# hpsim/OGL

Measured on AMD Instinct MI355X. Metric: cg_iters_per_sec, higher is better.
Workload: dtype f64

## Files before the change

### ogl_amd/csrc/kernels.hpp

```cpp
#pragma once
#include <hip/hip_runtime.h>

#include "common.hpp"

namespace ogl {

struct DevCriterion {
    double tolerance, rel_tol;
    int32_t min_iter, max_iter, frequency, export_res;
};

struct DevScalars {
    double rho, prev_rho, beta;
    double alpha, omega, gamma;
    double norm_factor;
    double init_res, res;
    double xbar;
    double sums[4];
    int32_t iter;
    int32_t stop;
    int32_t n_evals;
    int32_t stop_phase;
    int32_t stop_turn;
    int32_t comm_error;
// ... 286 lines not shown
void launch_cg_step2(hipStream_t st, int32_t n, double *x, double *r, const double *p,
                     const double *q, const double *inv_diag, double *part_rho, double *part_norm,
                     const DevScalars *s);

struct HaloPutFused;
void launch_cg_step1x(hipStream_t st, int32_t n, double *p, double *x, const double *r,
                      const double *inv_diag, const DevScalars *s, const HaloPutFused *put = nullptr);
void launch_cg_step2r(hipStream_t st, int32_t n, double *r, const double *q, const double *inv_diag,
                      double *part_rho, double *part_norm, const DevScalars *s, double *z_out = nullptr,
                      const HaloPutFused *put = nullptr);

void launch_cg_step1x_fin(hipStream_t st, int32_t n, double *p, double *x, const double *r, const double *inv_diag,
                          const DevScalars *sin, DevScalars *sout, const double *part_rho,
                          const double *part_norm, double *history, int first, const LeadBox &lead = LeadBox{},
                          double *p_out = nullptr, const PRing &ring = PRing{});
void launch_cg_step2r_fin(hipStream_t st, int32_t n, double *r, const double *q, const double *inv_diag,
                          double *part_rho, double *part_norm, const DevScalars *sin, DevScalars *sout,
                          const double *part_beta, double *z_out = nullptr,
                          const LeadBox &lead = LeadBox{});
struct HeldZ {
    unsigned long long *tagged = nullptr;
    int32_t grid = 0;
    int32_t early_slots = 0;
};
constexpr int HZ_B = 4, HZ_R = 11, HZ_L = 9;
int held_z_grid(int *chunks_per_workgroup);
int launch_resident_census(hipStream_t st, int grid, unsigned *arrived, int *out, long long timeout_ticks);
void launch_cg_step2r1x(hipStream_t st, int32_t n, double *r, const double *q, const double *inv_diag, double *p,
                        double *p_out, double *x, DevScalars *s, const double *part_beta, double *history,
                        const LeadBox &lead, const PRing &ring, const HeldZ &hz);
struct HeldQ {
    int32_t on = 0;
    int32_t n_pos = 0;
};
int held_q_positions(const DevSym &A);
int held_q_occupancy(int *per_cu, size_t *lds_bytes);
void launch_cg_turn_held_q(hipStream_t st, const DevSym &A, double *r, const double *inv_diag, double *p, double *p_out,
                           double *x, DevScalars *s, double *history, const LeadBox &lead, const PRing &ring,
                           const HeldZ &hz, const HeldQ &hq);
constexpr int FUSED_FIN_MAX_CHUNKS = 1024;
void launch_cg_turn_sym(hipStream_t st, const DevSym &A, const double *p_in, double *p_out, double *x, const double *z,
                        double *q, double *part_beta, const DevScalars *sin, DevScalars *sout,
                        const double *part_rho, const double *part_norm, double *history, int first,
                        const LeadBox &lead = LeadBox{});
void launch_cg_turn_sym_big(hipStream_t st, const DevSym &A, const double *p_in, double *p_out, double *x,
                            const double *z, double *q, double *part_beta, const DevScalars *s,
                            const HaloFused &hf = HaloFused{}, const double *p_halo_in = nullptr,
                            double *p_halo_out = nullptr);

void launch_gmres_mgs_fold(hipStream_t st, int32_t n, double *w, const double *vprev, double *h_out, const double *vdot,
                           const double *part_in, double *part_out, const DevScalars *gate, const LeadBox &lead = LeadBox{},
                           uint32_t tag = 0);
void launch_bicg_fold1(hipStream_t st, int32_t n, double *p, const double *r, const double *v, const double *inv_diag,
                       double *y, const DevScalars *sin, DevScalars *sout, const double *part_rho,
                       const double *part_norm, double *history, const LeadBox &lead = LeadBox{});
void launch_bicg_fold2(hipStream_t st, int32_t n, const double *r, const double *v, double *sv, const double *inv_diag,
                       double *z, double *part_norm_out, const DevScalars *sin, DevScalars *sout,
                       const double *part_beta, const LeadBox &lead = LeadBox{});
void launch_bicg_fold3(hipStream_t st, int32_t n, double *x, double *r, const double *sv, const double *t,
                       const double *y, const double *z, const double *rr, double *part_rho_out, double *part_norm_out,
                       const DevScalars *sin, DevScalars *sout, const double *part_gamma, const double *part_tt,
                       const double *part_snorm, double *history, int turn, const LeadBox &lead = LeadBox{});
void launch_bicg_step1(hipStream_t st, int32_t n, double *p, const double *r, const double *v,
                       const double *inv_diag, double *y, const DevScalars *s);
void launch_bicg_step2(hipStream_t st, int32_t n, const double *r, const double *v, double *sv,
                       const double *inv_diag, double *z, double *part_norm, const DevScalars *s);
void launch_bicg_step3(hipStream_t st, int32_t n, double *x, double *r, const double *sv,
// ... 140 lines not shown
```

### ogl_amd/csrc/kernels_spmv_sym.hip

```cpp
#include <algorithm>

#include "device_common.hpp"
#include "resident_cg_turn.hpp"

namespace ogl {

namespace {

struct SymOffsets {
    int d[SYM_MAX_OFFSETS];
};
SymOffsets sym_offsets(const DevSym &A, bool *fast)
{
    SymOffsets off;
    for (int j = 0; j < SYM_MAX_OFFSETS; ++j) off.d[j] = A.d[j];
    *fast = A.nd >= 2 && A.d[1] == 1;
    for (int j = 2; j < A.nd; ++j) *fast = *fast && (A.d[j] % 2 == 0);
    return off;
}
template <int MODE, int ND, bool FAST, bool STREAM>
__device__ __forceinline__ double2 sym_rows(int chunk, const RowPair &rp, int n_rows, const SymOffsets &off,
                                            const uint8_t *__restrict__ mask, const double *__restrict__ planes,
                                            const double *__restrict__ x, const double *__restrict__ b,
                                            double2 &xd_out)
// ... 341 lines not shown
        return;
    }
    const unsigned mm = *reinterpret_cast<const unsigned short *>(mask + rp.row);
    const unsigned m0 = mm & 0xffu, m1 = mm >> 8;
    TurnSymRegs<ND> R;
    turn_sym_load<ND, FAST, STREAM>(R, chunk, rp, n_rows, off, planes, p_in, z);
    if (pending) {
        const double beta = s->beta;
        if (beta != 0.0) {
            const double t = s->prev_rho / beta;
            double2 vx = ld2_stream(x, rp);
            vx.x += t * R.vd[0].x;
            vx.y += t * R.vd[0].y;
            st2_stream(x, rp, vx);
        }
    }
    const double rho = s->rho, prev = s->prev_rho;
    const double tmp = (prev == 0.0) ? 0.0 : rho / prev;
    double2 xd;
    double2 acc = turn_sym_rows<ND>(R, m0, m1, tmp, xd);
    st2(p_out, rp, xd);
    if (HALO) {
        __shared__ double ys[CHUNK_ROWS];
        if (hf.chunk_bptr) halo_fused_add<SPMV_PLAIN, true>(hf, chunk, acc.x, acc.y, ys, tmp, ph_in, ph_out);
    }
    st2(q, rp, acc);
    double d = 0.0;
    if (rp.n > 0) d += xd.x * acc.x;
    if (rp.n > 1) d += xd.y * acc.y;
    const double sd = block_sum(d, slot);
    if (threadIdx.x == 0) part_beta[chunk] = sd;
}

struct HeldQSrc {
    static constexpr bool Q_HELD = true;
    static constexpr int STRIDE = 6, WORD = 2;
    int G, n_pos, n_partials;
    const int *__restrict__ block_order;
    __device__ __forceinline__ int chunk_of(int i) const
    {
        const int pos = blockIdx.x + i * G;
        if (pos >= n_pos) return -1;
        const int c = block_order ? block_order[pos] : xcd_chunk(pos);
        return c < n_partials ? c : -1;
    }
};
template <int R, int L, int B, int K, int ND, bool FAST>
__global__ __launch_bounds__(BLOCK, B) void k_cg_turn_held_q(int n, int n_chunks, int n_pos, SymOffsets off,
                                                             const uint8_t *__restrict__ mask,
                                                             const double *__restrict__ planes,
                                                             const int *__restrict__ block_order, double *__restrict__ r,
                                                             const double *__restrict__ inv_diag, double *p, double *p_out,
                                                             double *__restrict__ x, DevScalars *s,
                                                             unsigned long long *tagged, double *history, LeadBox lead,
                                                             const double *p_pend, int ring_phase, int early_slots)
{
    __shared__ double zl[L > 0 ? L * CHUNK_ROWS : 1];
    __shared__ TurnLds lds;
    const TurnScalars ts = turn_prelude<K>(s, ring_phase);
    const TurnArgs a{n, r, inv_diag, p, p_out, x, s, tagged, history, lead, p_pend, early_slots};
    const HeldQSrc src{(int)gridDim.x, n_pos, n_chunks, block_order};
    const int G = gridDim.x, w = blockIdx.x;
    if (ts.stopped) return;
    TurnSlots<R, L> z;
    z.zl = zl;
#pragma unroll
    for (int i = 0; i < R + L; ++i) {
        const int chunk = src.chunk_of(i);
        if (chunk < 0) continue;
        const RowPair rp = my_rows(chunk, n);
        double2 xd;
        double2 vq = sym_rows<SPMV_PLAIN, ND, FAST, true>(chunk, rp, n, off, mask, planes, p, nullptr, xd);
        if (rp.n < 2) vq.y = 0.0;
        if (rp.n < 1) vq.x = 0.0;
        z.put(i, vq);
        double d = 0.0;
        if (rp.n > 0) d += xd.x * vq.x;
        if (rp.n > 1) d += xd.y * vq.y;
        const double sd = block_sum(d, lds.slot);
        if (threadIdx.x == 0) put_tagged(tagged + HeldQSrc::STRIDE * (size_t)chunk, ts.seq, sd);
    }
    const int lead0 = G >= 3 * FIN_WAVES ? 2 * FIN_WAVES : 0;
    if (w >= lead0 && w < lead0 + FIN_WAVES)
        lead_wave_sums_tagged(lead, ts.seq, tagged, HeldQSrc::STRIDE, n_chunks, w - lead0, 0);
    TurnFront<HeldQSrc::Q_HELD> f;
    turn_ask_first(src, a, f);
    double beta;
    if (!turn_await_beta(a, ts, lds, beta)) return;
    resident_cg_turn<R, L, K>(src, a, ts, lds, z, f, beta);
}

}

void launch_spmv_sym(hipStream_t st, const DevSym &A, int mode, const double *x, const double *b, double *y,
                     const SpmvDots &dots, const DevScalars *gate, const HaloFused &hf)
{
    if (A.n_rows == 0) return;
    const int nc = (int)n_chunks(A.n_rows);
    const dim3 grid(A.block_order ? A.n_blocks : xcd_grid(nc)), block(BLOCK);
    bool fast;
    const SymOffsets off = sym_offsets(A, &fast);
#define OGL_SYM_K(MODE, NDOT, ND, FAST, STREAM)                                                                          \
    hipLaunchKernelGGL((k_spmv_sym<MODE, NDOT, ND, FAST, STREAM>), grid, block, 0, st, A.n_rows, nc, off, A.mask, A.planes, \
                       x, b, y, dots.with, dots.part, dots.part_yy, gate, A.block_order, hf)
#define OGL_SYM_ND(MODE, NDOT, ND)                   \
    do {                                             \
        if (fast && A.stream)                        \
            OGL_SYM_K(MODE, NDOT, ND, true, true);   \
        else if (fast)                               \
            OGL_SYM_K(MODE, NDOT, ND, true, false);  \
        else if (A.stream)                           \
            OGL_SYM_K(MODE, NDOT, ND, false, true);  \
        else                                         \
            OGL_SYM_K(MODE, NDOT, ND, false, false); \
    } while (0)
#define OGL_SYM(MODE, NDOT)                    \
    do {                                       \
        if (A.nd == 2)                         \
// ... 67 lines not shown
    const SymOffsets off = sym_offsets(A, &fast);
#define OGL_TURN_K(ND, FAST, STREAM)                                                                                \
    do {                                                                                                            \
        if (hf.chunk_bptr)                                                                                          \
            hipLaunchKernelGGL((k_cg_turn_sym_big<ND, FAST, STREAM, true>), grid, block, 0, st, A.n_rows, nc, off,  \
                               A.mask, A.planes, p_in, p_out, x, z, q, part_beta, s, A.block_order, hf, p_halo_in,  \
                               p_halo_out);                                                                         \
        else                                                                                                        \
            hipLaunchKernelGGL((k_cg_turn_sym_big<ND, FAST, STREAM, false>), grid, block, 0, st, A.n_rows, nc, off, \
                               A.mask, A.planes, p_in, p_out, x, z, q, part_beta, s, A.block_order, HaloFused{},    \
                               nullptr, nullptr);                                                                   \
    } while (0)
#define OGL_TURN_ND(ND)                     \
    do {                                    \
        if (fast && A.stream)               \
            OGL_TURN_K(ND, true, true);     \
        else if (fast)                      \
            OGL_TURN_K(ND, true, false);    \
        else if (A.stream)                  \
            OGL_TURN_K(ND, false, true);    \
        else                                \
            OGL_TURN_K(ND, false, false);   \
    } while (0)
    if (A.nd == 2)
        OGL_TURN_ND(2);
    else if (A.nd == 3)
        OGL_TURN_ND(3);
    else
        OGL_TURN_ND(4);
#undef OGL_TURN_ND
#undef OGL_TURN_K
}

#define OGL_HELD_Q(K, ND, FAST) k_cg_turn_held_q<HZ_R, HZ_L, HZ_B, K, ND, FAST>
#define OGL_HELD_Q_EACH(DO) \
    DO(0, 2, false) DO(0, 2, true) DO(0, 3, false) DO(0, 3, true) DO(0, 4, false) DO(0, 4, true) \
    DO(2, 2, false) DO(2, 2, true) DO(2, 3, false) DO(2, 3, true) DO(2, 4, false) DO(2, 4, true)
int held_q_positions(const DevSym &A)
{
    return A.block_order ? A.n_blocks : xcd_grid((int)n_chunks(A.n_rows));
}

int held_q_occupancy(int *per_cu, size_t *lds_bytes)
{
    *per_cu = HZ_B;
    *lds_bytes = 0;
#define OGL_HELD_Q_ASK(K, ND, FAST)                                                                                  \
    {                                                                                                                \
        int o = 0;                                                                                                   \
        hipFuncAttributes fa;                                                                                        \
        if (hipOccupancyMaxActiveBlocksPerMultiprocessor(&o, OGL_HELD_Q(K, ND, FAST), BLOCK, 0) != hipSuccess ||     \
            hipFuncGetAttributes(&fa, reinterpret_cast<const void *>(OGL_HELD_Q(K, ND, FAST))) != hipSuccess)        \
            return 1;                                                                                                \
        *per_cu = std::min(*per_cu, o);                                                                              \
        *lds_bytes = std::max(*lds_bytes, (size_t)fa.sharedSizeBytes);                                               \
    }
    OGL_HELD_Q_EACH(OGL_HELD_Q_ASK)
#undef OGL_HELD_Q_ASK
    return 0;
}

void launch_cg_turn_held_q(hipStream_t st, const DevSym &A, double *r, const double *inv_diag, double *p, double *p_out,
                           double *x, DevScalars *s, double *history, const LeadBox &lead, const PRing &ring,
                           const HeldZ &hz, const HeldQ &hq)
{
    if (A.n_rows == 0) return;
    const int nc = (int)n_chunks(A.n_rows);
    const dim3 grid(hz.grid), block(BLOCK);
    bool fast;
    const SymOffsets off = sym_offsets(A, &fast);
#define OGL_HELD_Q_K(K, ND, FAST)                                                                                        \
    hipLaunchKernelGGL((OGL_HELD_Q(K, ND, FAST)), grid, block, 0, st, A.n_rows, nc, hq.n_pos, off, A.mask, A.planes,     \
                       A.block_order, r, inv_diag, p, K == 2 ? p_out : p, x, s, hz.tagged, history, lead,                \
                       K == 2 ? (const double *)ring.b[1] : nullptr, K == 2 ? ring.phase : 0, hz.early_slots)
#define OGL_HELD_Q_ND(K, ND)              \
    do {                                  \
        if (fast)                         \
            OGL_HELD_Q_K(K, ND, true);    \
        else                              \
            OGL_HELD_Q_K(K, ND, false);   \
    } while (0)
#define OGL_HELD_Q_RING(ND)         \
    do {                            \
        if (ring.k == 2)            \
            OGL_HELD_Q_ND(2, ND);   \
        else                        \
            OGL_HELD_Q_ND(0, ND);   \
    } while (0)
    static_assert(SYM_MAX_OFFSETS == 4, "instantiations above");
    if (A.nd == 2)
        OGL_HELD_Q_RING(2);
    else if (A.nd == 3)
        OGL_HELD_Q_RING(3);
    else
        OGL_HELD_Q_RING(4);
#undef OGL_HELD_Q_RING
#undef OGL_HELD_Q_ND
#undef OGL_HELD_Q_K
}
#undef OGL_HELD_Q_EACH
#undef OGL_HELD_Q

}
```

### ogl_amd/csrc/launch_key.hpp

```cpp
#pragma once
#include <cstdint>
#include <cstring>
#include <type_traits>

#include "kernels.hpp"

namespace ogl {

struct KeyHasher {
    uint64_t h = 1469598103934665603ull;
    void bytes(const void *p, size_t n)
    {
        const unsigned char *c = static_cast<const unsigned char *>(p);
        for (size_t i = 0; i < n; ++i) h = (h ^ c[i]) * 1099511628211ull;
    }
    template <class T>
    std::enable_if_t<std::is_arithmetic<T>::value || std::is_pointer<T>::value || std::is_enum<T>::value> operator()(const T &v)
    {
        bytes(&v, sizeof(v));
    }
};

#define OGL_VIEW_FIELDS(T, n)                                                                                        \
    static_assert(sizeof(T) == n, "a field of " #T " was added, removed or resized: bring visit(KeyHasher &, const " #T \
// ... 3 lines not shown
inline void visit(KeyHasher &h, const DevCsr &a)
{
    h(a.n_rows), h(a.nnz), h(a.row_ptrs), h(a.cols), h(a.vals), h(a.stream), h(a.xcd_group), h(a.chunks21), h(a.codes21);
    h(a.far_idx21), h(a.far_col21), h(a.block_order), h(a.n_blocks), h(a.lds_rounds);
}
OGL_VIEW_FIELDS(DevEll, 40);
inline void visit(KeyHasher &h, const DevEll &a)
{
    h(a.n_rows), h(a.width), h(a.stride), h(a.cols), h(a.vals), h(a.stream);
}
OGL_VIEW_FIELDS(DevSell, 112);
inline void visit(KeyHasher &h, const DevSell &a)
{
    h(a.n_rows), h(a.chunks), h(a.dict), h(a.codes), h(a.vals), h(a.spill_chunk_ptr), h(a.spill_rows), h(a.spill_ptrs);
    h(a.spill_cols), h(a.spill_vals), h(a.stream), h(a.xcd_group), h(a.rmap), h(a.block_order), h(a.n_blocks);
}
OGL_VIEW_FIELDS(DevSym, 64);
inline void visit(KeyHasher &h, const DevSym &a)
{
    h(a.n_rows), h(a.nd);
    for (int j = 0; j < 4; ++j) h(a.d[j]);
    h(a.mask), h(a.planes), h(a.stream), h(a.block_order), h(a.n_blocks);
}
OGL_VIEW_FIELDS(DevSymx, 96);
inline void visit(KeyHasher &h, const DevSymx &a)
{
    h(a.n_rows), h(a.chunks), h(a.chunks_general), h(a.n_blocks_general), h(a.mask), h(a.planes), h(a.ex_rowptr), h(a.ex_cols);
    h(a.ex_lrow), h(a.ex_vals), h(a.stream), h(a.fast), h(a.xcd_group), h(a.n_blocks);
}
OGL_VIEW_FIELDS(LeadBox, 24);
inline void visit(KeyHasher &h, const LeadBox &a) { h(a.box), h(a.timeout_ticks), h(a.early_loads); }
OGL_VIEW_FIELDS(HeldZ, 16);
inline void visit(KeyHasher &h, const HeldZ &a) { h(a.tagged), h(a.grid), h(a.early_slots); }
OGL_VIEW_FIELDS(HeldQ, 8);
inline void visit(KeyHasher &h, const HeldQ &a) { h(a.on), h(a.n_pos); }

#undef OGL_VIEW_FIELDS

}
```

### ogl_amd/csrc/resident_cg_turn.hpp

```cpp
#pragma once
#include "device_common.hpp"

namespace ogl {

namespace {

constexpr int TURN_AHEAD = 2;

struct TurnScalars {
    uint32_t seq;
    int stopped;
    double rho, norm_factor, init_res;
    int phase;
    bool defers;
    unsigned pending;
    double t1;
    int iter, n_evals;
    CritVals crit;
};
template <int K>
__device__ __forceinline__ TurnScalars turn_prelude(const DevScalars *s, int ring_phase)
{
    static_assert(K == 0 || K == 2, "p in place or two p buffers");
    TurnScalars t;
// ... 27 lines not shown
};

struct TurnLds {
    double sh[3];
    double slot[2 * N_WAVES];
    double lead_words[LEAD_BOX_WORDS / 2];
    int sh_stop;
    int lead_timed_out;
};

template <int R, int L>
struct TurnSlots {
    double2 zr[R];
    double *zl;
    __device__ __forceinline__ double2 get(int i) const
    {
        if (i < R) return zr[i < R ? i : 0];
        double2 v;
        v.x = zl[(i - R) * CHUNK_ROWS + ROWS_PER_THREAD * threadIdx.x];
        v.y = zl[(i - R) * CHUNK_ROWS + ROWS_PER_THREAD * threadIdx.x + 1];
        return v;
    }
    __device__ __forceinline__ void put(int i, const double2 &v)
    {
        if (i < R) {
            zr[i < R ? i : 0] = v;
        } else {
            zl[(i - R) * CHUNK_ROWS + ROWS_PER_THREAD * threadIdx.x] = v.x;
            zl[(i - R) * CHUNK_ROWS + ROWS_PER_THREAD * threadIdx.x + 1] = v.y;
        }
    }
};

__device__ __forceinline__ RowPair turn_rows(int chunk, int n)
{
    if (chunk >= 0) return my_rows(chunk, n);
    RowPair none;
    none.row = none.n = 0;
    return none;
}

template <bool Q_HELD>
struct TurnFront {
    double2 r[TURN_AHEAD], d[TURN_AHEAD], q[TURN_AHEAD];
};
template <>
struct TurnFront<true> {
    double2 r[TURN_AHEAD], d[TURN_AHEAD];
};
template <class Src>
__device__ __forceinline__ void turn_ask(const Src &src, const TurnArgs &a, TurnFront<Src::Q_HELD> &f, int i, int d)
{
    const RowPair rp = turn_rows(src.chunk_of(i), a.n);
    f.r[d] = ld2(a.r, rp);
    if constexpr (!Src::Q_HELD) f.q[d] = ld2_stream(src.q, rp);
    f.d[d].x = f.d[d].y = 1.0;
    if (a.inv_diag) f.d[d] = ld2_stream(a.inv_diag, rp);
}
template <class Src>
__device__ __forceinline__ void turn_ask_first(const Src &src, const TurnArgs &a, TurnFront<Src::Q_HELD> &f)
{
#pragma unroll
    for (int d = 0; d < TURN_AHEAD; ++d) turn_ask(src, a, f, d, d);
}

__device__ __forceinline__ bool turn_await_beta(const TurnArgs &a, const TurnScalars &ts, TurnLds &lds, double &beta)
// ... 57 lines not shown
        }
    }
    if (w < 2 * FIN_WAVES)
        lead_wave_sums_tagged(a.lead, tag, a.tagged + Src::WORD + 2 * (w / FIN_WAVES), Src::STRIDE, src.n_partials,
                              w % FIN_WAVES, 1 + w / FIN_WAVES);
}

template <int R, int L, int K, class Src>
__device__ __forceinline__ void turn_phase_h(const Src &src, const TurnArgs &a, const TurnScalars &ts, TurnLds &lds,
                                             const TurnSlots<R, L> &z, double beta)
{
    const int w = blockIdx.x;
    const uint32_t tag = ts.seq + 1;
    const bool own_term = beta != 0.0;
    const double t_own = own_term ? ts.rho / beta : 0.0;
    auto update_x = [&](const RowPair &rp, const double2 &vp, int upto) {
        const bool pend = K > 1 && 1 < upto && ((ts.pending >> 1) & 1u);
        if (!pend && !own_term) return;
        double2 vx = ld2_stream(a.x, rp);
        if (pend) {
            const double2 v1 = ld2(a.p_pend, rp);
            vx.x += ts.t1 * v1.x;
            vx.y += ts.t1 * v1.y;
        }
        if (own_term) {
            vx.x += t_own * vp.x;
            vx.y += t_own * vp.y;
        }
        st2_stream(a.x, rp, vx);
    };
    const int n_early = ts.defers ? 0 : min(a.early_slots, R + L);
#pragma unroll 2
    for (int i = 0; i < n_early; ++i) {
        const int chunk = src.chunk_of(i);
        if (chunk < 0) continue;
        const RowPair rp = my_rows(chunk, a.n);
        update_x(rp, ld2(a.p, rp), K);
    }
    if (!lead_wait(a.lead, 4 * FIN_WAVES, tag, lds.lead_words, &lds.lead_timed_out, 2 * FIN_WAVES)) {
        if (threadIdx.x == 0) a.s->comm_error = a.s->stop = 1;
        return;
    }
    if (threadIdx.x == 0) {
        const double prev_rho = ts.rho, rho = lead_total(lds.lead_words, 0), norm = lead_total(lds.lead_words, 1);
        const Verdict cv = criterion_verdict(ts.crit, ts.iter, ts.n_evals, ts.init_res, ts.norm_factor, norm,
                                             w == 0 ? a.history : nullptr);
        lds.sh[1] = prev_rho;
        lds.sh[2] = rho;
        lds.sh_stop = cv.stop;
        if (w == 0) {
            DevScalars *s = a.s;
            s->beta = beta;
            s->prev_rho = prev_rho;
            s->rho = rho;
            s->x_pending = 0;
            store_verdict(s, cv);
            s->launch_seq = ts.seq + 2;
            s->defer_valid = (ts.defers && !cv.stop) ? (int)(ts.pending | (own_term ? 1u << ts.phase : 0u)) : 0;
            if (ts.defers && own_term) s->t_ring[ts.phase] = t_own;
        }
    }
    __syncthreads();
    const double prev = lds.sh[1], rho = lds.sh[2];
    const int stop = lds.sh_stop;
    const double tmp = (prev == 0.0) ? 0.0 : rho / prev;
#pragma unroll
    for (int i = 0; i < R + L; ++i) {
// ... 26 lines not shown
```

### ogl_amd/csrc/solver.cpp

```cpp
#include "solver_internal.hpp"

#include "setup_kernels.hpp"

#include <algorithm>
#include <atomic>
#include <chrono>
#include <condition_variable>
#include <cmath>
#include <cstddef>
#include <cstring>
#include <future>
#if defined(__x86_64__)
#include <immintrin.h>
#endif
#include <sched.h>
#include <mutex>
#include <thread>

using namespace ogl;


namespace {
#if defined(__x86_64__)
__attribute__((target("avx2"))) void stream_copy_avx2(char *d, const char *s, size_t len)
// ... 175 lines not shown
ogl_registry::~ogl_registry()
{
    if (device >= 0) (void)hipSetDevice(device);
    if (stream) (void)hipStreamSynchronize(stream);
    solvers.clear();
    comm.reset();
    peer_close();
    cached_precond.release();
    if (comm_stream) {
        (void)hipStreamSynchronize(comm_stream);
        stream_destroy(comm_stream);
        ev_destroy(ev_packed);
        ev_destroy(ev_received);
    }
    if (own_stream && stream) stream_destroy(stream);
}

void ogl_solver::drop_cg_graph()
{
    if (cg_graph) {
        (void)hipGraphExecDestroy(cg_graph);
        ledger::destroyed(ledger::GRAPH_EXEC);
    }
    cg_graph = nullptr;
    cg_graph_key = 0;
}

ogl_solver::~ogl_solver()
{
    drop_cg_graph();
    ledger::pinned_free(h_scal);
    ledger::dev_free(lead_box);
    ledger::dev_free(held_z_box);
    mixed.release();
    for (auto &e : poll_ev)
        if (e) ev_destroy(e);
    for (auto &e : prof_ev)
        if (e) ev_destroy(e);
    for (auto &e : chk_ev)
        if (e) ev_destroy(e);
}

double ogl_solver::prop(const std::string &key, double dflt) const
{
    auto it = props.find(key);
    return it == props.end() ? dflt : it->second;
}

double ogl_solver::stream_above_bytes() const
{
    static const double env_default = [] {
        const char *e = std::getenv("OGL_STREAM_ABOVE_BYTES");
        return e ? atof(e) : STREAM_MATRIX_ABOVE_BYTES;
    }();
    return prop("streamAboveBytes", env_default);
}

double ogl_solver::turn_extra_bytes() const
{
    if (prop("streamTurnSet", 1.0) == 0.0) return 0.0;
    const double N = (double)pat.n_rows, nnz = (double)pat.local_nnz;
    double extra = 0.0;
    if (cfg.preconditioner == OGL_PRECOND_ISAI) extra += 10.0 * (nnz + N);
    if (cfg.preconditioner == OGL_PRECOND_GISAI) extra += 10.0 * nnz;
    if (cfg.preconditioner == OGL_PRECOND_BJ && cfg.max_block_size > 1) extra += 8.0 * cfg.max_block_size * N;
    if (cfg.preconditioner == OGL_PRECOND_IC) extra += 24.0 * (nnz + N) / 2.0;
// ... 980 lines not shown
```

### ogl_amd/csrc/solver.hpp

```cpp
#pragma once
#include <hip/hip_runtime.h>

#include <algorithm>
#include <map>
#include <memory>
#include <string>
#include <vector>

#include "comm.hpp"
#include "common.hpp"
#include "host_matrix.hpp"
#include "kernels.hpp"
#include "setup_kernels.hpp"
#include "spmv_layouts.hpp"

namespace ogl {

struct MgLevel {
    int32_t n = 0, nnz = 0, n_coarse = 0;
    bool own = true;
    DevBuf<int32_t> row_ptrs, cols;
    DevBuf<double> vals, inv_d;
    DevBuf<int32_t> agg, agg_ptr, agg_rows;
    DevBuf<double> b, xa, xb, t, r, p;
// ... 371 lines not shown
    ogl::DevBuf<double> d_p_halo;
    ogl::DevBuf<double> d_bj_tmp0, d_bj_tmp1;
    ogl::DevBuf<double> d_v, d_s, d_t, d_y, d_z, d_rr;
    ogl::DevBuf<double> d_V, d_gm;
    ogl::DevBuf<double> d_gs_part, d_gs_h;
    ogl::DevBuf<double> d_isai_tmp;
    ogl::DevBuf<double> d_fac_tmp[3];
    int generate_multigrid(ogl::PrecondData &P);
    void apply_multigrid(const double *in, double *out, const ogl::DevScalars *gate, double *dot_part);
    void mg_cycle(int level, const double *b, double *x, const ogl::DevScalars *gate, int &launches);
    void mg_product(int level, const double *x, double *y, const ogl::DevScalars *gate);
    int check_multigrid_keywords();
    int mg_tail_first = 0;
    bool precond_ready = false;
    uint64_t precond_serial = 0, precond_pat = 0;
    bool precond_current() const;
    std::vector<int32_t> fac_seg_fwd, fac_seg_bwd;
    ogl::DevBuf<double> d_part0, d_part1, d_part2;
    int64_t band_order_rows = 0;
    bool source_diag_valid = false;
    int64_t csr_band_rows = 0;
    uint64_t csr_band_pat = 0;
    int csr_band(int64_t *band);
    ogl::DevBuf<int32_t> d_band_order;
    ogl::DevBuf<double> d_part3, d_part4, d_part5;
    ogl::DevBuf<ogl::DevScalars> d_scal;
    ogl::DevBuf<double> d_history;
    ogl::DevScalars *h_scal = nullptr;
    hipEvent_t poll_ev[2] = {nullptr, nullptr};
    unsigned long long *lead_box = nullptr;
    unsigned long long *held_z_box = nullptr;
    size_t held_z_words = 0;
    int held_z_census = 0, held_z_census_grid = 0;
    hipEvent_t chk_ev[2] = {nullptr, nullptr};
    bool x_resident = false, b_resident = false;
    ogl::PrecondData own_precond;
    const ogl::PrecondData *precond_data = nullptr;
    const double *precond = nullptr;

    std::map<std::string, double> props;

    std::vector<double> history;
    double t_update_matrix_ms = 0;
    std::vector<hipEvent_t> prof_ev;

    ~ogl_solver();

    int set_matrix(const ogl_ldu_view &ldu);
    int solve(const double *source, double *psi, ogl_perf *perf);
    int apply_resident(ogl_perf *perf);
    int upload_vec(ogl::DevBuf<double> &dst, const double *src);
    int ensure_vectors();
    int init_preconditioner();
    int generate_preconditioner(ogl::PrecondData &P);
    int generate_jacobi(ogl::PrecondData &P);
    int generate_block_jacobi(ogl::PrecondData &P, bool through_perm);
    int generate_isai(ogl::PrecondData &P, bool caller_numbering);
    int generate_factor(ogl::PrecondData &P);
    int prepare_apply();
    void apply_factor(const double *in, double *out, const ogl::DevScalars *gate, double *dot_part);
    int check_factor_breakdown(int32_t word);
    void apply_preconditioner(const double *in, double *out, const ogl::DevScalars *gate,
                              double *dot_part = nullptr);
    int dist_spmv(int mode, const double *x, const double *b, double *y, const ogl::SpmvDots &dots,
                  const ogl::DevScalars *gate, bool prepacked = false);
    void spmv_on(ogl::SpmvLayout l, int mode, const double *x, const double *b, double *y, const ogl::SpmvDots &dots,
// ... 56 lines not shown
```

### ogl_amd/csrc/solver_krylov.cpp

```cpp
#include "launch_key.hpp"
#include "solver_internal.hpp"

#include <algorithm>
#include <cmath>
#include <cstring>
#include <vector>

using namespace ogl;

HaloPutFused ogl_solver::begin_halo_put()
{
    HaloPutFused put;
    if (!(pat.non_local_nnz > 0 && peer_halo) || prop("haloFused", 1.0) == 0.0 || peer_safe_wait())
        return put;
    if (++halo_seq == 0) ++halo_seq;
    cur_halo = peer_halo_args(halo_seq);
    put.P = cur_halo;
    put.chunk_sptr = d_chunk_sptr.p;
    put.send_pos = d_send_pos.p;
    put.send_idxs = d_send_idxs.p;
    put.ticket = d_ticket.p;
    put.n_put_chunks = n_put_chunks;
    return put;
}
// ... 629 lines not shown

int ogl_solver::turn_cg_held_z(KrylovRun &k, int enq, int pe)
{
    hipStream_t st = k.st;
    const int n = k.n;
    double *p_new = k.p_of_turn(enq + 1);
    if (enq == 0) {
        OGL_HIP_CHECK(hipEventRecord(k.ev_chk[0], st));
        launch_cg_step1x_fin(st, n, k.p_of_turn(0), d_x.p, d_r.p, precond, k.s, k.s2, d_part0.p, d_part1.p, d_history.p, 1,
                             k.lead, p_new, k.ring_of_turn(0));
        OGL_HIP_CHECK(hipEventRecord(k.ev_chk[1], st));
    }
    if (pe >= 0) OGL_HIP_CHECK(hipEventRecord(prof_ev[2 * pe], st));
    OGL_TRY(dist_spmv(SPMV_PLAIN, p_new, nullptr, d_q.p, SpmvDots{p_new, d_part2.p, nullptr}, k.s2));
    if (pe >= 0) OGL_HIP_CHECK(hipEventRecord(prof_ev[2 * pe + 1], st));
    launch_cg_step2r1x(st, n, d_r.p, d_q.p, precond, p_new, k.p_of_turn(enq + 2), d_x.p, k.s2, d_part2.p, d_history.p, k.lead,
                       k.ring_of_turn(enq + 1), k.hz);
    return OGL_OK;
}

int ogl_solver::turn_cg_held_q(KrylovRun &k, int enq, int pe)
{
    if (pe >= 0) return turn_cg_held_z(k, enq, pe);
    hipStream_t st = k.st;
    double *p_new = k.p_of_turn(enq + 1);
    if (enq == 0) {
        OGL_HIP_CHECK(hipEventRecord(k.ev_chk[0], st));
        launch_cg_step1x_fin(st, k.n, k.p_of_turn(0), d_x.p, d_r.p, precond, k.s, k.s2, d_part0.p, d_part1.p, d_history.p, 1,
                             k.lead, p_new, k.ring_of_turn(0));
        OGL_HIP_CHECK(hipEventRecord(k.ev_chk[1], st));
    }
    launch_cg_turn_held_q(st, sym(), d_r.p, precond, p_new, k.p_of_turn(enq + 2), d_x.p, k.s2, d_history.p, k.lead,
                          k.ring_of_turn(enq + 1), k.hz, k.hq);
    return OGL_OK;
}

int ogl_solver::plan_held_z(KrylovRun &k)
{
    k.hz = HeldZ{};
    k.hq = HeldQ{};
    props["heldQInUse"] = 0.0;
    props["heldZInUse"] = 0.0;
    props["heldZGridInUse"] = 0.0;
    if (!(k.lead.box != nullptr && k.fused && !k.fused2 && !k.generic && !k.multi && (k.ring.k == 0 || k.ring.k == 2)))
        return OGL_OK;
    bool streams = false;
    switch (spmv_layout) {
    case SpmvLayout::Ell: streams = ell().stream; break;
    case SpmvLayout::Sell: streams = sell().stream; break;
    case SpmvLayout::Sym: streams = sym().stream; break;
    case SpmvLayout::Symx: streams = symx().stream; break;
    default: streams = csr().stream; break;
    }
    if (prop("heldZ", streams ? 1.0 : 0.0) == 0.0 || held_z_census < 0) return OGL_OK;
    int per_wg = 0;
    int grid = held_z_grid(&per_wg);
    grid = std::min(grid, (int)prop("heldZGrid", (double)grid));
    if (grid < 2 * 16) return OGL_OK;
    const double cap = std::min((double)grid * per_wg, prop("heldZMaxChunks", (double)grid * per_wg));
    if ((double)k.nc > cap) return OGL_OK;
    bool held_q = false;
    int n_pos = 0;
    if (spmv_layout == SpmvLayout::Sym) {
        n_pos = held_q_positions(sym());
        held_q = prop("heldQ", sym().stream && grid % 8 == 0 ? 1.0 : 0.0) != 0.0 && (double)n_pos <= (double)grid * per_wg;
    }
    hipStream_t st = k.st;
    const size_t words = (held_q ? 6 : 4) * (size_t)k.nc;
    if (!held_z_box || held_z_words < words) {
        ledger::dev_free(held_z_box);
        held_z_box = nullptr;
        void *b = nullptr;
        OGL_HIP_CHECK(ledger::dev_malloc(&b, words * sizeof(unsigned long long), true));
        held_z_box = static_cast<unsigned long long *>(b);
        held_z_words = words;
    }
    OGL_HIP_CHECK(hipMemsetAsync(held_z_box, 0, held_z_words * sizeof(unsigned long long), st));
    if (held_z_census == 0 || held_z_census_grid < grid) {
        void *c = nullptr;
        OGL_HIP_CHECK(ledger::dev_malloc(&c, 2 * sizeof(int)));
        int timed_out = 1;
        const int rc = launch_resident_census(st, grid, static_cast<unsigned *>(c), static_cast<int *>(c) + 1,
                                              (long long)(prop("heldZCensusS", 1.0) * 1e8));
        hipError_t e = rc == 0 ? hipMemcpyAsync(&timed_out, static_cast<int *>(c) + 1, sizeof(int), hipMemcpyDeviceToHost, st)
                               : hipErrorUnknown;
        if (e == hipSuccess) e = hipStreamSynchronize(st);
        ledger::dev_free(c);
        if (e != hipSuccess) return fail(OGL_ERR_HIP, "census of the held-z grid failed: %s", hipGetErrorString(e));
        held_z_census = timed_out ? -1 : 1;
        held_z_census_grid = grid;
        if (timed_out) return OGL_OK;
    }
    k.hz.tagged = held_z_box;
    k.hz.grid = grid;
    const int early_slots = std::max(0, std::min(per_wg, (int)prop("heldZEarlySlots", 4.0)));
    k.hz.early_slots = prop("heldZEarlyX", 1.0) != 0.0 ? early_slots : 0;
    props["heldZInUse"] = 1.0;
    props["heldZGridInUse"] = (double)grid;
    if (held_q) {
        k.hq.on = 1;
        k.hq.n_pos = n_pos;
        props["heldQInUse"] = 1.0;
    }
    return OGL_OK;
}

int ogl_solver::turn_cg_merged(KrylovRun &k, int enq, int pe)
{
    hipStream_t st = k.st;
    const int n = k.n;
    DevScalars *s = k.s;
    if (pe >= 0) OGL_HIP_CHECK(hipEventRecord(prof_ev[2 * pe], st));
    if (k.merged_halo) {
        launch_cg_turn_sym_big(st, sym(), k.p_of_turn(enq), k.p_of_turn(enq + 1), d_x.p,
                               k.z_kept ? k.z_kept : d_r.p, d_q.p, d_part0.p, s,
                               halo_fused_args(cur_halo), k.p_halo_of_turn(enq), k.p_halo_of_turn(enq + 1));
    } else {
        launch_cg_turn_sym_big(st, sym(), k.p_of_turn(enq), k.p_of_turn(enq + 1), d_x.p,
                               k.z_kept ? k.z_kept : d_r.p, d_q.p, d_part0.p, s);
    }
    if (pe >= 0) OGL_HIP_CHECK(hipEventRecord(prof_ev[2 * pe + 1], st));
    OGL_TRY(finalize(FIN_BETA, k.f1));
    if (k.merged_halo) {
        const HaloPutFused put = begin_halo_put();
        launch_cg_step2r(st, n, d_r.p, d_q.p, precond, d_part0.p, d_part1.p, s, k.z_kept, &put);
    } else {
        launch_cg_step2r(st, n, d_r.p, d_q.p, precond, d_part0.p, d_part1.p, s, k.z_kept);
    }
    k.chk.turn = 1;
    OGL_TRY(finalize(FIN_CG_CHECK, k.chk));
    return OGL_OK;
}

int ogl_solver::turn_cg_five_launch(KrylovRun &k, int, int pe)
{
    hipStream_t st = k.st;
// ... 374 lines not shown
```

Measured before the change: 4884.

## Add dynamic work-stealing chunk draw to held-q CG turn kernel

The held-q resident CG turn kernel now gives each workgroup a fixed number of static chunk slots and lets it claim the remaining chunks dynamically. Claims go through per-XCD atomic ticket counters, which are double-buffered by a parity bit that flips every turn. This is meant to balance load across workgroups so that tail imbalance in the SpMV phase shrinks. In exchange it adds atomics, extra __syncthreads, LDS bookkeeping and a larger R template, all of which could raise latency or cut occupancy.

```diff
diff --git a/ogl_amd/csrc/kernels.hpp b/ogl_amd/csrc/kernels.hpp
--- a/ogl_amd/csrc/kernels.hpp
+++ b/ogl_amd/csrc/kernels.hpp
@@ -342,7 +342,14 @@
 struct HeldQ {
     int32_t on = 0;
     int32_t n_pos = 0;
-};
+    int32_t static_slots = 0;
+    int32_t drawers = 0;
+    unsigned *heads = nullptr;
+    int32_t parity = 0;
+};
+constexpr int HQ_R = 13, HQ_STATIC = HZ_R + HZ_L;
+constexpr int HQ_STATIC_DEFAULT = 12;
+constexpr int HQ_HEAD_STRIDE = 32, HQ_HEAD_WORDS = 2 * N_XCD * HQ_HEAD_STRIDE;
 int held_q_positions(const DevSym &A);
 int held_q_occupancy(int *per_cu, size_t *lds_bytes);
 void launch_cg_turn_held_q(hipStream_t st, const DevSym &A, double *r, const double *inv_diag, double *p, double *p_out,
diff --git a/ogl_amd/csrc/kernels_spmv_sym.hip b/ogl_amd/csrc/kernels_spmv_sym.hip
--- a/ogl_amd/csrc/kernels_spmv_sym.hip
+++ b/ogl_amd/csrc/kernels_spmv_sym.hip
@@ -397,20 +397,32 @@
     if (threadIdx.x == 0) part_beta[chunk] = sd;
 }
 
+template <bool DRAW>
 struct HeldQSrc {
     static constexpr bool Q_HELD = true;
     static constexpr int STRIDE = 6, WORD = 2;
     int G, n_pos, n_partials;
     const int *__restrict__ block_order;
+    int S;
+    const int *drawn;
+    __device__ __forceinline__ int chunk_at(int pos) const
+    {
+        if (pos < 0 || pos >= n_pos) return -1;
+        const int c = block_order ? block_order[pos] : xcd_chunk(pos);
+        return c < n_partials ? c : -1;
+    }
     __device__ __forceinline__ int chunk_of(int i) const
     {
-        const int pos = blockIdx.x + i * G;
-        if (pos >= n_pos) return -1;
-        const int c = block_order ? block_order[pos] : xcd_chunk(pos);
-        return c < n_partials ? c : -1;
+        if constexpr (!DRAW) return chunk_at((int)blockIdx.x + i * G);
+        return chunk_at(i < S ? (int)blockIdx.x + i * G : __builtin_amdgcn_readfirstlane(drawn[i]));
+    }
+    __device__ __forceinline__ int chunk_of_rolled(int i) const
+    {
+        if constexpr (!DRAW) return chunk_at((int)blockIdx.x + i * G);
+        return chunk_at(i < S ? (int)blockIdx.x + i * G : drawn[i]);
     }
 };
-template <int R, int L, int B, int K, int ND, bool FAST>
+template <int R, int L, int B, int K, int ND, bool FAST, bool DRAW>
 __global__ __launch_bounds__(BLOCK, B) void k_cg_turn_held_q(int n, int n_chunks, int n_pos, SymOffsets off,
                                                              const uint8_t *__restrict__ mask,
                                                              const double *__restrict__ planes,
@@ -418,21 +430,50 @@
                                                              const double *__restrict__ inv_diag, double *p, double *p_out,
                                                              double *__restrict__ x, DevScalars *s,
                                                              unsigned long long *tagged, double *history, LeadBox lead,
-                                                             const double *p_pend, int ring_phase, int early_slots)
+                                                             const double *p_pend, int ring_phase, int early_slots,
+                                                             int static_slots, int drawers, unsigned *heads, int parity)
 {
     __shared__ double zl[L > 0 ? L * CHUNK_ROWS : 1];
     __shared__ TurnLds lds;
+    __shared__ int drawn[DRAW ? R + L : 1];
+    using Src = HeldQSrc<DRAW>;
     const TurnScalars ts = turn_prelude<K>(s, ring_phase);
     const TurnArgs a{n, r, inv_diag, p, p_out, x, s, tagged, history, lead, p_pend, early_slots};
-    const HeldQSrc src{(int)gridDim.x, n_pos, n_chunks, block_order};
     const int G = gridDim.x, w = blockIdx.x;
+    const int S = DRAW ? static_slots : R + L;
+    const Src src{G, n_pos, n_chunks, block_order, S, drawn};
     if (ts.stopped) return;
+    unsigned *const head = heads + (size_t)(parity * N_XCD + w % N_XCD) * HQ_HEAD_STRIDE;
+    const int q0 = S * G + ((w % N_XCD) - (S * G) % N_XCD + N_XCD) % N_XCD;
+    auto ask = [&]() { return __hip_atomic_fetch_add(head, 1u, __ATOMIC_RELAXED, __HIP_MEMORY_SCOPE_AGENT); };
+    auto position = [&](unsigned ticket) {
+        const long long pos = q0 + (long long)N_XCD * ticket;
+        return pos < n_pos ? (int)pos : -1;
+    };
+    bool more = DRAW && w < drawers;
+    if constexpr (DRAW) {
+        if (threadIdx.x < R + L) drawn[threadIdx.x] = -1;
+        if (w == 0 && threadIdx.x < N_XCD) heads[(size_t)((parity ^ 1) * N_XCD + threadIdx.x) * HQ_HEAD_STRIDE] = 0u;
+        if (more && S == 0 && threadIdx.x == 0) drawn[0] = position(ask());
+        __syncthreads();
+        if (more && S == 0) more = __builtin_amdgcn_readfirstlane(drawn[0]) >= 0;
+    }
     TurnSlots<R, L> z;
     z.zl = zl;
 #pragma unroll
     for (int i = 0; i < R + L; ++i) {
+        const bool ahead = DRAW && more && i + 1 >= S && i + 1 < R + L;
+        unsigned ticket = 0;
+        if (ahead && threadIdx.x == 0) ticket = ask();
         const int chunk = src.chunk_of(i);
-        if (chunk < 0) continue;
+        if (chunk < 0) {
+            if (ahead) {
+                if (threadIdx.x == 0) drawn[i + 1] = position(ticket);
+                __syncthreads();
+                more = __builtin_amdgcn_readfirstlane(drawn[i + 1]) >= 0;
+            }
+            continue;
+        }
         const RowPair rp = my_rows(chunk, n);
         double2 xd;
         double2 vq = sym_rows<SPMV_PLAIN, ND, FAST, true>(chunk, rp, n, off, mask, planes, p, nullptr, xd);
@@ -442,13 +483,15 @@
         double d = 0.0;
         if (rp.n > 0) d += xd.x * vq.x;
         if (rp.n > 1) d += xd.y * vq.y;
+        if (ahead && threadIdx.x == 0) drawn[i + 1] = position(ticket);
         const double sd = block_sum(d, lds.slot);
-        if (threadIdx.x == 0) put_tagged(tagged + HeldQSrc::STRIDE * (size_t)chunk, ts.seq, sd);
+        if (ahead) more = __builtin_amdgcn_readfirstlane(drawn[i + 1]) >= 0;
+        if (threadIdx.x == 0) put_tagged(tagged + Src::STRIDE * (size_t)chunk, ts.seq, sd);
     }
     const int lead0 = G >= 3 * FIN_WAVES ? 2 * FIN_WAVES : 0;
     if (w >= lead0 && w < lead0 + FIN_WAVES)
-        lead_wave_sums_tagged(lead, ts.seq, tagged, HeldQSrc::STRIDE, n_chunks, w - lead0, 0);
-    TurnFront<HeldQSrc::Q_HELD> f;
+        lead_wave_sums_tagged(lead, ts.seq, tagged, Src::STRIDE, n_chunks, w - lead0, 0);
+    TurnFront<Src::Q_HELD> f;
     turn_ask_first(src, a, f);
     double beta;
     if (!turn_await_beta(a, ts, lds, beta)) return;
@@ -582,7 +625,7 @@
 #undef OGL_TURN_K
 }
 
-#define OGL_HELD_Q(K, ND, FAST) k_cg_turn_held_q<HZ_R, HZ_L, HZ_B, K, ND, FAST>
+#define OGL_HELD_Q(K, ND, FAST, DRAW) k_cg_turn_held_q<DRAW ? HQ_R : HZ_R, HZ_L, HZ_B, K, ND, FAST, DRAW>
 #define OGL_HELD_Q_EACH(DO) \
     DO(0, 2, false) DO(0, 2, true) DO(0, 3, false) DO(0, 3, true) DO(0, 4, false) DO(0, 4, true) \
     DO(2, 2, false) DO(2, 2, true) DO(2, 3, false) DO(2, 3, true) DO(2, 4, false) DO(2, 4, true)
@@ -595,18 +638,20 @@
 {
     *per_cu = HZ_B;
     *lds_bytes = 0;
-#define OGL_HELD_Q_ASK(K, ND, FAST)                                                                                  \
-    {                                                                                                                \
-        int o = 0;                                                                                                   \
-        hipFuncAttributes fa;                                                                                        \
-        if (hipOccupancyMaxActiveBlocksPerMultiprocessor(&o, OGL_HELD_Q(K, ND, FAST), BLOCK, 0) != hipSuccess ||     \
-            hipFuncGetAttributes(&fa, reinterpret_cast<const void *>(OGL_HELD_Q(K, ND, FAST))) != hipSuccess)        \
-            return 1;                                                                                                \
-        *per_cu = std::min(*per_cu, o);                                                                              \
-        *lds_bytes = std::max(*lds_bytes, (size_t)fa.sharedSizeBytes);                                               \
-    }
+#define OGL_HELD_Q_ASK_ONE(K, ND, FAST, DRAW)                                                                            \
+    {                                                                                                                    \
+        int o = 0;                                                                                                       \
+        hipFuncAttributes fa;                                                                                            \
+        if (hipOccupancyMaxActiveBlocksPerMultiprocessor(&o, OGL_HELD_Q(K, ND, FAST, DRAW), BLOCK, 0) != hipSuccess ||   \
+            hipFuncGetAttributes(&fa, reinterpret_cast<const void *>(OGL_HELD_Q(K, ND, FAST, DRAW))) != hipSuccess)      \
+            return 1;                                                                                                    \
+        *per_cu = std::min(*per_cu, o);                                                                                  \
+        *lds_bytes = std::max(*lds_bytes, (size_t)fa.sharedSizeBytes);                                                   \
+    }
+#define OGL_HELD_Q_ASK(K, ND, FAST) OGL_HELD_Q_ASK_ONE(K, ND, FAST, false) OGL_HELD_Q_ASK_ONE(K, ND, FAST, true)
     OGL_HELD_Q_EACH(OGL_HELD_Q_ASK)
 #undef OGL_HELD_Q_ASK
+#undef OGL_HELD_Q_ASK_ONE
     return 0;
 }
 
@@ -620,9 +665,17 @@
     bool fast;
     const SymOffsets off = sym_offsets(A, &fast);
 #define OGL_HELD_Q_K(K, ND, FAST)                                                                                        \
-    hipLaunchKernelGGL((OGL_HELD_Q(K, ND, FAST)), grid, block, 0, st, A.n_rows, nc, hq.n_pos, off, A.mask, A.planes,     \
+    do {                                                                                                                 \
+        if (hq.static_slots < HQ_STATIC)                                                                                 \
+            OGL_HELD_Q_KD(K, ND, FAST, true);                                                                            \
+        else                                                                                                             \
+            OGL_HELD_Q_KD(K, ND, FAST, false);                                                                           \
+    } while (0)
+#define OGL_HELD_Q_KD(K, ND, FAST, DRAW)                                                                                 \
+    hipLaunchKernelGGL((OGL_HELD_Q(K, ND, FAST, DRAW)), grid, block, 0, st, A.n_rows, nc, hq.n_pos, off, A.mask, A.planes,     \
                        A.block_order, r, inv_diag, p, K == 2 ? p_out : p, x, s, hz.tagged, history, lead,                \
-                       K == 2 ? (const double *)ring.b[1] : nullptr, K == 2 ? ring.phase : 0, hz.early_slots)
+                       K == 2 ? (const double *)ring.b[1] : nullptr, K == 2 ? ring.phase : 0, hz.early_slots,            \
+                       hq.static_slots, hq.drawers, hq.heads, hq.parity)
 #define OGL_HELD_Q_ND(K, ND)              \
     do {                                  \
         if (fast)                         \
@@ -646,6 +699,7 @@
         OGL_HELD_Q_RING(4);
 #undef OGL_HELD_Q_RING
 #undef OGL_HELD_Q_ND
+#undef OGL_HELD_Q_KD
 #undef OGL_HELD_Q_K
 }
 #undef OGL_HELD_Q_EACH
diff --git a/ogl_amd/csrc/launch_key.hpp b/ogl_amd/csrc/launch_key.hpp
--- a/ogl_amd/csrc/launch_key.hpp
+++ b/ogl_amd/csrc/launch_key.hpp
@@ -59,8 +59,11 @@
 inline void visit(KeyHasher &h, const LeadBox &a) { h(a.box), h(a.timeout_ticks), h(a.early_loads); }
 OGL_VIEW_FIELDS(HeldZ, 16);
 inline void visit(KeyHasher &h, const HeldZ &a) { h(a.tagged), h(a.grid), h(a.early_slots); }
-OGL_VIEW_FIELDS(HeldQ, 8);
-inline void visit(KeyHasher &h, const HeldQ &a) { h(a.on), h(a.n_pos); }
+OGL_VIEW_FIELDS(HeldQ, 32);
+inline void visit(KeyHasher &h, const HeldQ &a)
+{
+    h(a.on), h(a.n_pos), h(a.static_slots), h(a.drawers), h(a.heads), h(a.parity);
+}
 
 #undef OGL_VIEW_FIELDS
 
diff --git a/ogl_amd/csrc/resident_cg_turn.hpp b/ogl_amd/csrc/resident_cg_turn.hpp
--- a/ogl_amd/csrc/resident_cg_turn.hpp
+++ b/ogl_amd/csrc/resident_cg_turn.hpp
@@ -83,6 +83,17 @@
     }
 };
 
+template <class Src>
+__device__ __forceinline__ auto turn_chunk_rolled(const Src &src, int i, int) -> decltype(src.chunk_of_rolled(i))
+{
+    return src.chunk_of_rolled(i);
+}
+template <class Src>
+__device__ __forceinline__ int turn_chunk_rolled(const Src &src, int i, long)
+{
+    return src.chunk_of(i);
+}
+
 __device__ __forceinline__ RowPair turn_rows(int chunk, int n)
 {
     if (chunk >= 0) return my_rows(chunk, n);
@@ -206,7 +217,7 @@
     const int n_early = ts.defers ? 0 : min(a.early_slots, R + L);
 #pragma unroll 2
     for (int i = 0; i < n_early; ++i) {
-        const int chunk = src.chunk_of(i);
+        const int chunk = turn_chunk_rolled(src, i, 0);
         if (chunk < 0) continue;
         const RowPair rp = my_rows(chunk, a.n);
         update_x(rp, ld2(a.p, rp), K);
diff --git a/ogl_amd/csrc/solver.cpp b/ogl_amd/csrc/solver.cpp
--- a/ogl_amd/csrc/solver.cpp
+++ b/ogl_amd/csrc/solver.cpp
@@ -231,6 +231,7 @@
     ledger::pinned_free(h_scal);
     ledger::dev_free(lead_box);
     ledger::dev_free(held_z_box);
+    ledger::dev_free(held_q_heads);
     mixed.release();
     for (auto &e : poll_ev)
         if (e) ev_destroy(e);
diff --git a/ogl_amd/csrc/solver.hpp b/ogl_amd/csrc/solver.hpp
--- a/ogl_amd/csrc/solver.hpp
+++ b/ogl_amd/csrc/solver.hpp
@@ -427,6 +427,7 @@
     unsigned long long *held_z_box = nullptr;
     size_t held_z_words = 0;
     int held_z_census = 0, held_z_census_grid = 0;
+    unsigned *held_q_heads = nullptr;
     hipEvent_t chk_ev[2] = {nullptr, nullptr};
     bool x_resident = false, b_resident = false;
     ogl::PrecondData own_precond;
diff --git a/ogl_amd/csrc/solver_krylov.cpp b/ogl_amd/csrc/solver_krylov.cpp
--- a/ogl_amd/csrc/solver_krylov.cpp
+++ b/ogl_amd/csrc/solver_krylov.cpp
@@ -685,6 +685,7 @@
     }
     launch_cg_turn_held_q(st, sym(), d_r.p, precond, p_new, k.p_of_turn(enq + 2), d_x.p, k.s2, d_history.p, k.lead,
                           k.ring_of_turn(enq + 1), k.hz, k.hq);
+    if (k.hq.static_slots < HQ_STATIC) k.hq.parity ^= 1;
     return OGL_OK;
 }
 
@@ -693,6 +694,8 @@
     k.hz = HeldZ{};
     k.hq = HeldQ{};
     props["heldQInUse"] = 0.0;
+    props["heldQStaticSlotsInUse"] = 0.0;
+    props["heldQSlotsPerGroup"] = 0.0;
     props["heldZInUse"] = 0.0;
     props["heldZGridInUse"] = 0.0;
     if (!(k.lead.box != nullptr && k.fused && !k.fused2 && !k.generic && !k.multi && (k.ring.k == 0 || k.ring.k == 2)))
@@ -753,8 +756,35 @@
     if (held_q) {
         k.hq.on = 1;
         k.hq.n_pos = n_pos;
+        k.hq.static_slots = HQ_STATIC;
+        k.hq.drawers = grid;
         props["heldQInUse"] = 1.0;
-    }
+        const int slots = HQ_R + HZ_L;
+        const int S = std::max(0, std::min(HQ_STATIC, (int)prop("heldQStaticSlots", (double)HQ_STATIC_DEFAULT)));
+        const int idle = (int)prop("heldQIdleGroups", 0.0);
+        const int drawers = (S == 0 && idle > 0 && idle % N_XCD == 0 && idle < grid) ? grid - idle : grid;
+        bool fits = (long long)S * grid < n_pos;
+        for (int q = 0; fits && q < N_XCD; ++q) {
+            auto members = [q](long long lo, long long hi) {
+                auto below = [q](long long v) { return v <= q ? 0 : (v - q + N_XCD - 1) / N_XCD; };
+                return hi > lo ? below(hi) - below(lo) : 0;
+            };
+            fits = members(0, drawers) * (slots - S) >= members((long long)S * grid, n_pos);
+        }
+        if (fits) {
+            if (!held_q_heads) {
+                void *h = nullptr;
+                OGL_HIP_CHECK(ledger::dev_malloc(&h, HQ_HEAD_WORDS * sizeof(unsigned)));
+                held_q_heads = static_cast<unsigned *>(h);
+            }
+            OGL_HIP_CHECK(hipMemsetAsync(held_q_heads, 0, HQ_HEAD_WORDS * sizeof(unsigned), st));
+            k.hq.static_slots = S;
+            k.hq.drawers = drawers;
+            k.hq.heads = held_q_heads;
+        }
+    }
+    props["heldQStaticSlotsInUse"] = (double)k.hq.static_slots;
+    props["heldQSlotsPerGroup"] = !k.hq.on ? 0.0 : (double)((k.hq.static_slots < HQ_STATIC ? HQ_R : HZ_R) + HZ_L);
     return OGL_OK;
 }
 
```

New measurement: 5019 (median of 6 runs). 2.8% higher.
